# quanpn90/avsr

Measured on AMD Instinct MI355X. Metric: AV-frames/sec/GPU (fwd+bwd) on 15s clips; WER parity on LRS2 test, higher is better.
Workload: dtype bf16

## Files before the change

avsr_amd/_lib.py:

```python
import ctypes
import os

import torch

_HERE = os.path.dirname(os.path.abspath(__file__))
LIB_PATH = os.environ.get("AVSR_LIB_PATH_AB") or os.path.join(_HERE, "libavsr_hip.so")

AVSR_F32, AVSR_BF16 = 0, 1
ACT_NONE, ACT_GELU, ACT_RELU = 0, 1, 2

_c_p = ctypes.c_void_p
_i64 = ctypes.c_int64
_f = ctypes.c_float
_i = ctypes.c_int


class GemmParams(ctypes.Structure):
    _fields_ = [
        ("M", _i), ("N", _i), ("K", _i), ("batch", _i),
        ("dtype", _i), ("a_kmajor", _i), ("b_kmajor", _i), ("c_f32", _i),
        ("A", _c_p), ("lda", _i64), ("strideA", _i64),
        ("B", _c_p), ("ldb", _i64), ("strideB", _i64),
        ("C", _c_p), ("ldc", _i64), ("strideC", _i64),
        ("alpha", _f), ("beta", _f),
# ... 367 lines not shown
    global _lib
    if _lib is not None:
        return _lib
    if not os.path.exists(LIB_PATH):
        raise AvsrLibError(f"{LIB_PATH} not built: run `python -c 'import __graft_entry__ as g; g.build()'`")
    lib = ctypes.CDLL(LIB_PATH, mode=ctypes.RTLD_GLOBAL)
    for name, (argtypes, restype) in SYMBOLS.items():
        if os.environ.get("AVSR_LIB_PATH_AB") and not hasattr(lib, name):
            continue
        fn = getattr(lib, name)
        fn.argtypes = argtypes
        fn.restype = restype
    _lib = lib
    return lib


def check(rc, op):
    if rc != 0:
        raise AvsrLibError(f"{op} failed with code {rc}")


OPTIONS = {"gemm_tile": 0, "attn_sq_fwd": 1, "attn_sq_bwd": 2, "wgrad_dual": 3, "conv_192": 4, "conv_s2phase": 5,
           "conv_patch": 6, "conv_wpatch": 7, "stem_pool_2x2": 8,
           "stem_wpatch": 9, "attn_enc_fused": 10}
TILES = ["128", "256", "256x128", "128x256", "128s3", "128w8s3", "pp", "192", "192x256", "192w8s3", "64", "64s4"]
ATTN_PATHS = ["f32", "tiled", "resident", "sq", "enc"]
CONV_PATHS = ["reg", "glds", "patch", "s2", "wpatch", "stem_wpatch"]
CONV_PASSES = ["fwd", "dgrad", "wgrad"]


def set_option(name, value):
    if name == "gemm_tile" and not isinstance(value, int):
        value = 0 if value in (None, "auto") else TILES.index(value) + 1
    lib = load()
    prev = get_option(name)
    check(lib.avsr_set_option(OPTIONS[name], int(value)), f"avsr_set_option({name}, {value})")
    return prev


def get_option(name):
    return int(load().avsr_get_option(OPTIONS[name]))


_raw_stream = getattr(torch._C, "_cuda_getCurrentRawStream", None)
_get_device = getattr(torch._C, "_cuda_getDevice", None) or torch.cuda.current_device


def stream_ptr(device=None):
    if _raw_stream is not None:
        idx = _get_device() if device is None else torch.device(device).index
# ... 5 lines not shown
```

avsr_amd/csrc/conv.h:

```cpp
#pragma once
#include "gemm_core.h"
#include "gemm_glds.h"

namespace conv {
using namespace gemmcore;
using gemmg::GBK;
using gemmg::OOB;
using gemmg::bglds16;
using gemmg::make_rsrc;

struct ConvArgs {
  ConvGeom g;
  uint32_t a_bytes, b_bytes;
  const void* a; const void* b;
  int64_t a_gstride, b_gstride, c_gstride;
  int M, N, K, splits, kchunk;
  float* ws;
  Epi e;
  gemmg::BnrArgs bnr;
};

enum { K_FWD = 0, K_DGRAD = 1, K_WGRAD = 2, K_DGRAD_BNR = 3 };

struct WgradPlan { int splits, kchunk; bool slab; };
struct ConvPlan {
  int path, bm, tiles;
  int cls_bm[4], cls_tiles[4];
  uint32_t a_bytes, b_bytes;
  WgradPlan w;
  int64_t ws_floats;
};

constexpr int PATCH_ROWS = 384;
using PCfg = gemmg::GCfg<4, 1, 2, 2, 3>;
constexpr int WP_BLOCKS = 128, WP_COLS = 576, SWP_BLOCKS = 256, SWP_COLS = 392;

template <int R, int NW> struct BWgtR {
  static constexpr bool KMAJ = false;
  static constexpr int CPR = R / 8, RPP = 64 / CPR, SLOTS = GBK / RPP / NW;
  __amdgpu_buffer_rsrc_t rs; ConvGeom g;
  uint32_t vo[SLOTS];
  AVSR_DEV void init(const bf16* base, uint32_t bytes, const ConvGeom& g_, int r0, int rext, int wave, int lane) {
    rs = make_rsrc(base, bytes); g = g_;
    const int ktot = g.ktot_w;
#pragma unroll
    for (int i = 0; i < SLOTS; ++i) {
      const int pc = i * NW + wave, pk = pc * RPP + lane / CPR;
      const int r = r0 + ((lane % CPR) ^ gemmg::rswz<CPR>(pk)) * 8;
      vo[i] = r < rext ? (uint32_t)(((int64_t)pk * ktot + r) * 2) : OOB;
    }
  }
  AVSR_DEV void issue(char* img, int k0, int wave) const {
    const int ktot = g.ktot_w;
    int tap = k0 >> g.cout_shift;
    if (g.tap_step != 1) {
      const int u = (int)fdiv(tap, g.f_kw), v = tap - u * (int)g.f_kw.d;
      tap = (g.tap_kh0 + g.tap_step * u) * g.tap_kfw + g.tap_kw0 + g.tap_step * v;
    }
    const uint32_t so = (uint32_t)((((int64_t)(k0 & ((1 << g.cout_shift) - 1))) * ktot + (int64_t)tap * g.cin) * 2);
#pragma unroll
    for (int i = 0; i < SLOTS; ++i) bglds16(rs, vo[i], so, img + (i * NW + wave) * 1024);
  }
};

int igemm_f32(int kind, int bm, const ConvArgs& a, int groups, hipStream_t st);
int igemm_glds(int kind, int bm, const ConvArgs& a, int groups, hipStream_t st);
int patch_launch(int kind, const ConvArgs& a, const avsr_conv_params* p, hipStream_t st);
int wpatch_launch(const avsr_conv_params* p, hipStream_t st);
int stem_wpatch_launch(const avsr_conv_params* p, hipStream_t st);
int wgrad_reduce(float* ws, int splits, int chunks, int64_t mn, int groups, float* dw, int64_t dw_gstride, hipStream_t st);
}
```

avsr_amd/csrc/conv.hip:

```cpp
#include "conv.h"

namespace conv {
namespace {

int ilog2(int v) { int s = 0; while ((1 << s) < v) ++s; return (1 << s) == v ? s : -1; }

int make_geom(const avsr_conv_params* p, ConvGeom& g) {
  g.nimg = p->nimg; g.hin = p->hin; g.win = p->win; g.hout = p->hout; g.wout = p->wout;
  g.kh = p->kh; g.kw = p->kw; g.sh = p->sh; g.sw = p->sw; g.ph = p->ph; g.pw = p->pw;
  g.cin = p->cin; g.cout = p->cout; g.ldx = p->ldx; g.ldy = p->ldy;
  g.f_hw_out = make_fastdiv((uint32_t)(p->hout * p->wout));
  g.f_w_out = make_fastdiv((uint32_t)p->wout);
  g.f_hw_in = make_fastdiv((uint32_t)(p->hin * p->win));
  g.f_w_in = make_fastdiv((uint32_t)p->win);
  g.f_kw = make_fastdiv((uint32_t)p->kw);
  g.cin_shift = ilog2(p->cin); g.cout_shift = ilog2(p->cout);
  g.ktot_w = p->kh * p->kw * p->cin; g.tap_kfw = p->kw; g.tap_kh0 = 0; g.tap_kw0 = 0; g.tap_step = 1;
  const int ve = p->dtype == AVSR_BF16 ? 8 : 4;
  if (g.cin_shift < 0 || g.cout_shift < 0 || p->cin < ve || p->cout < ve) return AVSR_E_SHAPE;
  if (p->ldx % ve || p->ldy % ve) return AVSR_E_ALIGN;
  if (p->groups < 1 || p->ldx < (int64_t)p->groups * p->cin || p->ldy < (int64_t)p->groups * p->cout) return AVSR_E_SHAPE;
  return 0;
}

// ... 64 lines not shown
  const int64_t W = p->win, HW = (int64_t)p->hin * p->win, Wp = W + 2;
  const int64_t span = (PCfg::BM - 1) + 2 * ((PCfg::BM - 1) / W + 1) + 2 * Wp * ((PCfg::BM - 1) / HW + 1) + 2 * (Wp + 1) + 1;
  return span <= PATCH_ROWS;
}

bool wpatch_ok(const avsr_conv_params* p) {
  if (!avsr_opt(AVSR_OPT_CONV_WPATCH) || p->groups != 1 || p->splitk > 0) return false;
  if (p->kh != 3 || p->kw != 3 || p->sh != 1 || p->sw != 1 || p->ph != 1 || p->pw != 1) return false;
  if (p->cin != p->cout || p->ldx != p->cin || p->ldy != p->cout || p->hin != p->hout || p->win != p->wout) return false;
  if (p->hin != p->win) return false;
  const int64_t bytes = (int64_t)p->nimg * p->hin * p->win * p->cin * 2;
  if (bytes <= 0 || bytes >= (int64_t)OOB - (1 << 20)) return false;
  return (p->cin == 64 && p->hin == 22) || (p->cin == 128 && p->hin == 11) || (p->cin == 256 && p->hin == 6) ||
         (p->cin == 512 && p->hin == 3);
}

bool stem_wpatch_ok(const avsr_conv_params* p) {
  if (!avsr_opt(AVSR_OPT_STEM_WPATCH) || p->groups != 1 || p->splitk > 0) return false;
  if (p->cin != 8 || p->ldx != 8 || p->cout != 64 || p->ldy != 64 || p->kh != 7 || p->kw != 7) return false;
  if (p->sh != 2 || p->sw != 2 || p->ph != 3 || p->pw != 3 || p->hin != 88 || p->win != 88) return false;
  if (p->hout != 44 || p->wout != 44) return false;
  const int64_t dyb = (int64_t)p->nimg * 1936 * 128;
  return dyb > 0 && dyb < (int64_t)OOB - (1 << 20);
}

int conv_plan(const avsr_conv_params* p, int pass, ConvPlan& pl) {
  if (p->dtype != AVSR_BF16 && p->dtype != AVSR_F32) return AVSR_E_DTYPE;
  const bool bf = p->dtype == AVSR_BF16;
  pl = ConvPlan{};
  pl.path = bf ? AVSR_CONV_PATH_GLDS : AVSR_CONV_PATH_REG;
  const int64_t ktot = (int64_t)p->kh * p->kw * p->cin, ew = p->cout * ktot;
  const int64_t ex = ((int64_t)p->nimg * p->hin * p->win - 1) * p->ldx + p->cin;
  const int64_t ey = ((int64_t)p->nimg * p->hout * p->wout - 1) * p->ldy + p->cout;
  if (pass == AVSR_CONV_WGRAD) {
    set_extents(pl, bf, ey, ex);
    pl.bm = row_tile(p->cout, (int)ktot, p->groups, false);
    if (p->nimg * p->hout * p->wout == 0) return 0;
    const WgradPlan sized = wgrad_plan(p, pl.bm, bf, true);
    const int patch = !bf ? 0 : wpatch_ok(p) ? AVSR_CONV_PATH_WPATCH : stem_wpatch_ok(p) ? AVSR_CONV_PATH_STEM_WPATCH : 0;
    pl.ws_floats = patch == AVSR_CONV_PATH_WPATCH        ? (int64_t)WP_BLOCKS * 64 * WP_COLS
                   : patch == AVSR_CONV_PATH_STEM_WPATCH ? (int64_t)SWP_BLOCKS * 64 * SWP_COLS
                   : sized.slab                          ? (int64_t)p->groups * sized.splits * p->cout * ktot
                                                         : 0;
    if (p->ws && patch) pl.path = patch;
    pl.w = p->ws ? sized : wgrad_plan(p, pl.bm, bf, false);
    return 0;
  }
  const bool fwd = pass == AVSR_CONV_FWD;
  const int M = p->nimg * (fwd ? p->hout * p->wout : p->hin * p->win), N = fwd ? p->cout : p->cin;
  if (fwd) set_extents(pl, bf && (p->cin % 64) == 0, ex, ew);
  else set_extents(pl, bf && (p->cout % 64) == 0 && (p->sh == 1 || p->sh == 2) && p->sw == p->sh, ey, ew);
  if (!fwd && s2_phase(p, pl)) {
    pl.path = AVSR_CONV_PATH_S2;
    S2Class cl[4];
    s2_classes(p, cl);
    for (int q = 0; q < 4; ++q) {
      const int Mc = p->nimg * cl[q].hc * cl[q].wc;
      pl.cls_bm[q] = row_tile(Mc, N, 1, true);
      pl.cls_tiles[q] = (Mc + pl.cls_bm[q] - 1) / pl.cls_bm[q];
      pl.tiles += pl.cls_tiles[q];
    }
    return 0;
  }
  if (patch_ok(p, pl) && !(fwd && (p->bias || p->act || p->res || p->preact))) {
    pl.path = AVSR_CONV_PATH_PATCH;
    pl.bm = PCfg::BM;
  } else {
    pl.bm = row_tile(M, N, p->groups, bf);
  }
  pl.tiles = (M + pl.bm - 1) / pl.bm;
  return 0;
}

__global__ __launch_bounds__(256) void wgrad_reduce_kernel(float* ws, int splits, int chunks, int64_t mn,
                                                           float* dw, int64_t dw_gstride) {
  const int g = blockIdx.y, c = blockIdx.z;
  float* w = ws + (int64_t)g * splits * mn;
  float* d = dw + (int64_t)g * dw_gstride;
  const int nch = chunks < 0 ? -chunks : chunks;
  for (int64_t i = ((int64_t)blockIdx.x * 256 + threadIdx.x) * 4; i < mn; i += (int64_t)gridDim.x * 1024) {
    f32x4 s = {0.f, 0.f, 0.f, 0.f};
    if (chunks < 0) {
      for (int q = 0; q < nch; ++q) s += *(const f32x4*)(w + (int64_t)((int64_t)splits * q / nch) * mn + i);
    } else {
      const int s0 = (int)((int64_t)splits * c / chunks), s1 = (int)((int64_t)splits * (c + 1) / chunks);
      for (int q = s0; q < s1; ++q) s += *(const f32x4*)(w + (int64_t)q * mn + i);
      if (chunks > 1) {
        *(f32x4*)(w + (int64_t)s0 * mn + i) = s;
        continue;
// ... 1 lines not shown
    }
#pragma unroll
    for (int r = 0; r < 4; ++r) d[i + r] += s[r];
  }
}

int s2_launch(int kind, const ConvArgs& a0, const avsr_conv_params* p, const ConvPlan& pl, hipStream_t st) {
  S2Class cl[4];
  s2_classes(p, cl);
  int64_t tile_off = 0;
  for (int q = 0; q < 4; ++q) {
    const S2Class& k = cl[q];
    const int Mc = p->nimg * k.hc * k.wc;
    if (Mc == 0) continue;
    ConvArgs a = a0;
    a.g.hin = k.hc; a.g.win = k.wc; a.g.kh = k.nkh; a.g.kw = k.nkw; a.g.sh = 1; a.g.sw = 1;
    a.g.ph = k.ci; a.g.pw = k.cj;
    a.g.f_hw_in = make_fastdiv((uint32_t)(k.hc * k.wc));
    a.g.f_w_in = make_fastdiv((uint32_t)k.wc);
    a.g.f_kw = make_fastdiv((uint32_t)(k.nkw > 0 ? k.nkw : 1));
    a.g.tap_kh0 = k.kh0; a.g.tap_kw0 = k.kw0; a.g.tap_step = 2;
    a.M = Mc; a.K = k.nkh * k.nkw * p->cout; a.kchunk = a.K;
    a.e.M = Mc;
    a.e.rm_wc = k.wc; a.e.rm_hc = k.hc; a.e.rm_hin = p->hin; a.e.rm_win = p->win; a.e.rm_a = k.a; a.e.rm_b = k.b;
    if (kind >= K_DGRAD_BNR) a.bnr.ws = a0.bnr.ws + tile_off * 4 * a.N;
    tile_off += pl.cls_tiles[q];
    if (kind == K_DGRAD && a.K == 0 && a.e.beta == 1.f) continue;
    const int rc = igemm_glds(kind, pl.cls_bm[q], a, 1, st);
    if (rc) return rc;
  }
  return 0;
}

bool query_plan(const avsr_conv_params* p, int pass, ConvPlan& pl) { return p && conv_plan(p, pass, pl) == 0; }

}

int wgrad_reduce(float* ws, int splits, int chunks, int64_t mn, int groups, float* dw, int64_t dw_gstride, hipStream_t st) {
  const int xb = avsr_grid(mn / 4, 256, 1024);
  hipLaunchKernelGGL(wgrad_reduce_kernel, dim3((unsigned)xb, (unsigned)groups, (unsigned)chunks), dim3(256), 0, st, ws,
                     splits, chunks, mn, dw, dw_gstride);
  AVSR_CHECK_LAUNCH();
  if (chunks > 1) {
    hipLaunchKernelGGL(wgrad_reduce_kernel, dim3((unsigned)xb, (unsigned)groups, 1u), dim3(256), 0, st, ws, splits,
                       -chunks, mn, dw, dw_gstride);
    AVSR_CHECK_LAUNCH();
  }
  return 0;
}
}
using namespace conv;

extern "C" int avsr_conv_path(const avsr_conv_params* p, int pass) {
  if (!p || pass < AVSR_CONV_FWD || pass > AVSR_CONV_WGRAD) return AVSR_E_ARG;
  ConvGeom g;
  ConvPlan pl;
  int rc = make_geom(p, g);
  if (!rc) rc = conv_plan(p, pass, pl);
  return rc ? rc : pl.path;
}

extern "C" int avsr_conv_stat_tiles(const avsr_conv_params* p) {
  ConvPlan pl;
  return query_plan(p, AVSR_CONV_FWD, pl) ? pl.tiles : 0;
}

extern "C" int avsr_conv_bnr_tiles(const avsr_conv_params* p) {
  ConvPlan pl;
  return query_plan(p, AVSR_CONV_DGRAD, pl) ? pl.tiles : 0;
}

extern "C" int64_t avsr_conv_wgrad_ws(const avsr_conv_params* p) {
  ConvPlan pl;
  return query_plan(p, AVSR_CONV_WGRAD, pl) ? pl.ws_floats : 0;
}

extern "C" int avsr_conv_fwd(const avsr_conv_params* p, void* stream) {
  if (!p) return AVSR_E_ARG;
  ConvArgs a{};
  int rc = make_geom(p, a.g);
  if (rc) return rc;
  if (!avsr_aligned16(p->x) || !avsr_aligned16(p->w) || !avsr_aligned16(p->y)) return AVSR_E_ALIGN;
  if (p->stats && p->groups != 1) return AVSR_E_ARG;
  a.a = p->x; a.b = p->w;
  a.a_gstride = p->cin; a.b_gstride = (int64_t)p->cout * p->kh * p->kw * p->cin; a.c_gstride = p->cout;
  a.M = p->nimg * p->hout * p->wout; a.N = p->cout; a.K = p->kh * p->kw * p->cin;
  a.splits = 1; a.kchunk = a.K;
  a.e.M = a.M; a.e.N = a.N; a.e.C = p->y; a.e.ldc = p->ldy; a.e.alpha = 1.f; a.e.stats = p->stats;
  a.e.bias = p->bias; a.e.act = p->act; a.e.preact = p->preact; a.e.res = p->res; a.e.ldr = p->ldy;
  if (p->stats && (p->bias || p->act || p->res)) return AVSR_E_ARG;
  if (a.M == 0) return 0;
  ConvPlan pl;
  if ((rc = conv_plan(p, AVSR_CONV_FWD, pl))) return rc;
  a.a_bytes = pl.a_bytes; a.b_bytes = pl.b_bytes; a.e.stats_tiles = pl.tiles;
  hipStream_t st = (hipStream_t)stream;
  switch (pl.path) {
    case AVSR_CONV_PATH_REG: return igemm_f32(K_FWD, pl.bm, a, p->groups, st);
    case AVSR_CONV_PATH_PATCH: return patch_launch(K_FWD, a, p, st);
    default: return igemm_glds(K_FWD, pl.bm, a, p->groups, st);
  }
}

extern "C" int avsr_conv_bwd_data(const avsr_conv_params* p, void* stream) {
  if (!p) return AVSR_E_ARG;
  ConvArgs a{};
  int rc = make_geom(p, a.g);
  if (rc) return rc;
  if (!avsr_aligned16(p->dx) || !avsr_aligned16(p->w) || !avsr_aligned16(p->dy)) return AVSR_E_ALIGN;
  a.a = p->dy; a.b = p->w;
  a.a_gstride = p->cout; a.b_gstride = (int64_t)p->cout * p->kh * p->kw * p->cin; a.c_gstride = p->cin;
  a.M = p->nimg * p->hin * p->win; a.N = p->cin; a.K = p->kh * p->kw * p->cout;
  a.splits = 1; a.kchunk = a.K;
  a.e.M = a.M; a.e.N = a.N; a.e.C = p->dx; a.e.ldc = p->ldx; a.e.alpha = p->alpha; a.e.beta = p->beta;
  int kind = K_DGRAD;
  if (p->bnr_h) {
    if (p->dtype != AVSR_BF16 || p->groups != 1 || !p->bnr_ws || !p->bnr_scale ||
        !p->bnr_shift || !p->bnr_prelu || !p->bnr_mean || !p->bnr_invstd || (p->bnr_scale2 && !p->bnr_res) ||
        (p->bnr_scale2 && (!p->bnr_shift2 || !p->bnr_mean2 || !p->bnr_invstd2)))
      return AVSR_E_ARG;
    if (!avsr_aligned16(p->bnr_h) || (p->bnr_res && !avsr_aligned16(p->bnr_res))) return AVSR_E_ALIGN;
    a.bnr.h = (const bf16*)p->bnr_h; a.bnr.res = (const bf16*)p->bnr_res;
    a.bnr.scale = p->bnr_scale; a.bnr.shift = p->bnr_shift; a.bnr.prelu = p->bnr_prelu;
    a.bnr.mean = p->bnr_mean; a.bnr.invstd = p->bnr_invstd; a.bnr.scale2 = p->bnr_scale2;
    a.bnr.shift2 = p->bnr_shift2; a.bnr.mean2 = p->bnr_mean2; a.bnr.invstd2 = p->bnr_invstd2; a.bnr.ws = p->bnr_ws;
    kind = K_DGRAD_BNR + (p->bnr_scale2 ? 2 : p->bnr_res ? 1 : 0);
  }
  if (a.M == 0) return 0;
  ConvPlan pl;
  if ((rc = conv_plan(p, AVSR_CONV_DGRAD, pl))) return rc;
  a.a_bytes = pl.a_bytes; a.b_bytes = pl.b_bytes;
  hipStream_t st = (hipStream_t)stream;
  switch (pl.path) {
    case AVSR_CONV_PATH_REG: return igemm_f32(kind, pl.bm, a, p->groups, st);
    case AVSR_CONV_PATH_S2: return s2_launch(kind, a, p, pl, st);
    case AVSR_CONV_PATH_PATCH: return patch_launch(kind, a, p, st);
    default: return igemm_glds(kind, pl.bm, a, p->groups, st);
  }
}

extern "C" int avsr_conv_bwd_weight(const avsr_conv_params* p, void* stream) {
  if (!p) return AVSR_E_ARG;
  ConvArgs a{};
  int rc = make_geom(p, a.g);
  if (rc) return rc;
  if (!avsr_aligned16(p->x) || !avsr_aligned16(p->dy) || !p->dw) return AVSR_E_ALIGN;
  a.a = p->dy; a.b = p->x;
  const int64_t ktot = (int64_t)p->kh * p->kw * p->cin;
  a.a_gstride = p->cout; a.b_gstride = p->cin; a.c_gstride = p->cout * ktot;
  a.M = p->cout; a.N = (int)ktot; a.K = p->nimg * p->hout * p->wout;
  if (a.K == 0) return 0;
  ConvPlan pl;
  if ((rc = conv_plan(p, AVSR_CONV_WGRAD, pl))) return rc;
  hipStream_t st = (hipStream_t)stream;
  if (pl.path == AVSR_CONV_PATH_WPATCH) return wpatch_launch(p, st);
  if (pl.path == AVSR_CONV_PATH_STEM_WPATCH) return stem_wpatch_launch(p, st);
  const WgradPlan& w = pl.w;
  a.a_bytes = pl.a_bytes; a.b_bytes = pl.b_bytes;
  a.splits = w.splits; a.kchunk = w.kchunk;
// ... 15 lines not shown
```

avsr_amd/csrc/conv_igemm.hip:

```cpp
#include "conv.h"

namespace conv {
namespace {

template <typename T, typename OutT, int WM, int WN, int KIND>
__global__ __launch_bounds__(NT) void conv_kernel(ConvArgs a) {
  extern __shared__ __attribute__((aligned(16))) char smem[];
  using TL = Tile<T, WM, WN>;
  const int z = blockIdx.z, grp = z / a.splits, sp = z % a.splits;
  const int m0 = blockIdx.y * TL::BM, n0 = blockIdx.x * TL::BN;
  const T* pa = (const T*)a.a + (int64_t)grp * a.a_gstride;
  const T* pb = (const T*)a.b + (int64_t)grp * a.b_gstride;
  f32x16 acc[2][2];
  const int kbeg = sp * a.kchunk, kend = min(a.K, kbeg + a.kchunk);
  if constexpr (KIND == K_FWD) {
    LdConvK<T, TL::BM, false> la; la.p = pa; la.g = a.g; la.rext = a.M; la.K = a.K;
    LdDenseK<T, TL::BN> lb; lb.p = pb; lb.ld = a.K; lb.rext = a.N; lb.K = a.K;
    mainloop<T, WM, WN>(la, lb, m0, n0, kbeg, kend, acc, smem);
  } else if constexpr (KIND == K_DGRAD) {
    LdConvK<T, TL::BM, true> la; la.p = pa; la.g = a.g; la.rext = a.M; la.K = a.K;
    LdWgtR<T, TL::BN> lb; lb.p = pb; lb.g = a.g; lb.rext = a.N; lb.K = a.K;
    mainloop<T, WM, WN>(la, lb, m0, n0, kbeg, kend, acc, smem);
  } else {
    LdDenseR<T, TL::BM> la; la.p = pa; la.ld = a.g.ldy; la.rext = a.M; la.K = a.K;
// ... 172 lines not shown
      const uint32_t h = fdiv(rem, g.f_w_in), w = rem - h * g.f_w_in.d;
      th0[i] = h + g.ph; tw0[i] = w + g.pw;
      ro[i] = (int)(((int64_t)n * g.hout * g.wout * g.ldy + kc) * 2);
    }
  }
  AVSR_DEV void issue(char* img, int k0, int wave) const {
    const int khw = k0 >> g.cout_shift, cb = k0 & ((1 << g.cout_shift) - 1);
    const int kh = (int)fdiv(khw, g.f_kw), kw = khw - kh * (int)g.f_kw.d;
    const int ldy2 = (int)g.ldy * 2, cb2 = cb * 2;
#pragma unroll
    for (int i = 0; i < SLOTS; ++i) {
      const int th = th0[i] - kh, tw = tw0[i] - kw;
      bool ok;
      int pix;
      if (g.sh == 1) {
        ok = (unsigned)th < (unsigned)g.hout && (unsigned)tw < (unsigned)g.wout;
        pix = th * g.wout + tw;
      } else {
        ok = ((th | tw) & 1) == 0 && (unsigned)(th >> 1) < (unsigned)g.hout && (unsigned)(tw >> 1) < (unsigned)g.wout;
        pix = (th >> 1) * g.wout + (tw >> 1);
      }
      bglds16(rs, ok ? (uint32_t)(ro[i] + pix * ldy2 + cb2) : OOB, 0u, img + (i * NW + wave) * 1024);
    }
  }
};

template <int R, int NW> struct BConvR {
  static constexpr bool KMAJ = false;
  static constexpr int CPR = R / 8, RPP = 64 / CPR, SLOTS = GBK / RPP / NW;
  __amdgpu_buffer_rsrc_t rs; ConvGeom g; int kend;
  int kr[SLOTS], rk[SLOTS], rw[SLOTS], rc[SLOTS];
  AVSR_DEV void init(const bf16* base, uint32_t bytes, const ConvGeom& g_, int r0, int rext, int kend_, int wave, int lane) {
    rs = make_rsrc(base, bytes); g = g_; kend = kend_;
#pragma unroll
    for (int i = 0; i < SLOTS; ++i) {
      const int pc = i * NW + wave, pk = pc * RPP + lane / CPR;
      const int r = r0 + ((lane % CPR) ^ gemmg::rswz<CPR>(pk)) * 8;
      kr[i] = pk;
      if (r >= rext) { rk[i] = -1000000; rw[i] = 0; rc[i] = 0; continue; }
      const int c = r & ((1 << g.cin_shift) - 1), khw = r >> g.cin_shift;
      const int kh = fdiv(khw, g.f_kw);
      rk[i] = kh - g.ph; rw[i] = khw - kh * g.f_kw.d - g.pw; rc[i] = c * 2;
    }
  }
  AVSR_DEV void issue(char* img, int k0, int wave) const {
    const int ldx2 = (int)g.ldx * 2;
// ... 45 lines not shown
    gemmg::mainloop_glds<CF>(la, lb, kbeg, nk, acc, smem);
  } else if constexpr (KIND == K_DGRAD || KIND >= K_DGRAD_BNR) {
    GConvK<CF::BM, CF::NW, true> la; la.init(pa, a.g, m0, a.M, kend, wave, lane);
    GWgtR<CF::BN, CF::NW> lb; lb.init(pb, a.g, n0, a.N, kend, wave, lane);
    gemmg::mainloop_glds<CF>(la, lb, kbeg, nk, acc, smem);
  } else {
    gemmg::GDenseR<CF::BM, CF::NW> la; la.init(pa, a.g.ldy, m0, a.M, kend, wave, lane);
    GConvR<CF::BN, CF::NW> lb; lb.init(pb, a.g, n0, a.N, kend, wave, lane);
    gemmg::mainloop_glds<CF>(la, lb, kbeg, nk, acc, smem);
  }
  if constexpr (KIND >= K_DGRAD_BNR) {
    gemmg::epilogue_bnr<CF, KIND - K_DGRAD_BNR>(a.e, a.bnr, m0, n0, acc, smem);
    return;
  }
  Epi e = a.e;
  if (KIND == K_WGRAD && a.ws) e.C = a.ws + ((int64_t)grp * a.splits + sp) * a.M * a.N;
  else e.C = (OutT*)e.C + (int64_t)grp * a.c_gstride;
  if (e.res) e.res = (const bf16*)e.res + (int64_t)grp * a.c_gstride;
  if (e.preact) e.preact = (bf16*)e.preact + (int64_t)grp * a.c_gstride;
  if (e.bias) e.bias += (int64_t)grp * a.c_gstride;
  gemmg::epilogue_g<bf16, OutT, CF>(e, m0, n0, acc, smem);
}

using CCfg128 = gemmg::GCfg<2, 2, 2, 2, 2>;
using CCfg256x64 = gemmg::GCfg<4, 1, 2, 2, 2>;
using CCfg64x256 = gemmg::GCfg<1, 4, 2, 2, 2>;
using CCfg192 = gemmg::GCfg<2, 2, 3, 2, 2>;

template <typename OutT, int KIND, class CF>
int launch_glds(const ConvArgs& a, int groups, hipStream_t st) {
  const int tm = (a.M + CF::BM - 1) / CF::BM, tn = (a.N + CF::BN - 1) / CF::BN;
  if (a.e.stats && a.e.stats_tiles != tm) return AVSR_E_SHAPE;
  const long nwg = (long)tm * tn * groups * a.splits;
  if (nwg > 0x7fffffffL) return AVSR_E_SHAPE;
  hipLaunchKernelGGL((conv_glds_kernel<OutT, KIND, CF>), dim3((unsigned)nwg), dim3(CF::NTH), CF::LDS_BYTES, st, a,
                     tm, tn);
  AVSR_CHECK_LAUNCH();
  return 0;
}

template <typename OutT, int KIND>
int glds_by_tile(int bm, const ConvArgs& a, int groups, hipStream_t st) {
  if constexpr (KIND != K_WGRAD) {
    if (bm == 192) return launch_glds<OutT, KIND, CCfg192>(a, groups, st);
  }
  if (bm == 256) return launch_glds<OutT, KIND, CCfg256x64>(a, groups, st);
  if (bm == 64) return launch_glds<OutT, KIND, CCfg64x256>(a, groups, st);
  return bm == 128 ? launch_glds<OutT, KIND, CCfg128>(a, groups, st) : AVSR_E_ARG;
}

template <typename T, typename OutT, int WM, int WN, int KIND>
int launch(const ConvArgs& a, int groups, hipStream_t st) {
  using TL = Tile<T, WM, WN, KIND != K_WGRAD, KIND == K_FWD>;
  dim3 grid((a.N + TL::BN - 1) / TL::BN, (a.M + TL::BM - 1) / TL::BM, groups * a.splits);
  if (a.e.stats && a.e.stats_tiles != (int)grid.y) return AVSR_E_SHAPE;
  if (grid.y > 65535) return AVSR_E_SHAPE;
  hipLaunchKernelGGL((conv_kernel<T, OutT, WM, WN, KIND>), grid, dim3(NT), TL::LDS_BYTES, st, a);
  AVSR_CHECK_LAUNCH();
  return 0;
}

template <int KIND>
int f32_by_tile(int bm, const ConvArgs& a, int groups, hipStream_t st) {
  if (bm == 256) return launch<float, float, 4, 1, KIND>(a, groups, st);
  if (bm == 64) return launch<float, float, 1, 4, KIND>(a, groups, st);
  return bm == 128 ? launch<float, float, 2, 2, KIND>(a, groups, st) : AVSR_E_ARG;
}

}

int igemm_f32(int kind, int bm, const ConvArgs& a, int groups, hipStream_t st) {
  if (kind == K_FWD) return f32_by_tile<K_FWD>(bm, a, groups, st);
  if (kind == K_DGRAD) return f32_by_tile<K_DGRAD>(bm, a, groups, st);
  return kind == K_WGRAD ? f32_by_tile<K_WGRAD>(bm, a, groups, st) : AVSR_E_ARG;
}

int igemm_glds(int kind, int bm, const ConvArgs& a, int groups, hipStream_t st) {
  switch (kind) {
    case K_FWD: return glds_by_tile<bf16, K_FWD>(bm, a, groups, st);
    case K_DGRAD: return glds_by_tile<bf16, K_DGRAD>(bm, a, groups, st);
    case K_WGRAD: return glds_by_tile<float, K_WGRAD>(bm, a, groups, st);
    case K_DGRAD_BNR: return glds_by_tile<bf16, K_DGRAD_BNR>(bm, a, groups, st);
    case K_DGRAD_BNR + 1: return glds_by_tile<bf16, K_DGRAD_BNR + 1>(bm, a, groups, st);
    case K_DGRAD_BNR + 2: return glds_by_tile<bf16, K_DGRAD_BNR + 2>(bm, a, groups, st);
    default: return AVSR_E_ARG;
  }
}
}
```

avsr_amd/csrc/gemm_core.h:

```cpp
#pragma once
#include "common.h"

namespace gemmcore {

constexpr int BKE = 32, NT = 256;

template <typename T> struct V { static constexpr int VE = 16 / (int)sizeof(T); static constexpr int ROW = BKE + VE; };

AVSR_DEV void zero(v16& v) { v.w[0] = v.w[1] = v.w[2] = v.w[3] = 0u; }

struct ConvGeom {
  int nimg, hin, win, hout, wout;
  int kh, kw, sh, sw, ph, pw;
  int cin, cout;
  int64_t ldx, ldy;
  FastDiv f_hw_out, f_w_out;
  FastDiv f_hw_in, f_w_in;
  FastDiv f_kw;
  int cin_shift, cout_shift;
  int ktot_w, tap_kfw, tap_kh0, tap_kw0, tap_step;
};

template <typename T, int R> struct LdDenseK {
  static constexpr bool KMAJ = true;
// ... 234 lines not shown
          }
        }
    }
    if (more) {
      lstore<T, TL::BM, LA::KMAJ>(lA + (cur ^ 1) * TL::SA, ra, tid);
      lstore<T, TL::BN, LB::KMAJ>(lB + (cur ^ 1) * TL::SB, rb, tid);
    }
    __syncthreads();
  }
}

struct Epi {
  int M, N;
  void* C; int64_t ldc;
  float alpha, beta;
  const float* bias;
  int act, bwd, atomic;
  void* preact;
  const void* res; int64_t ldr;
  const void* gate;
  float drop_p; uint64_t seed; uint64_t drop_base;
  float* stats;
  int stats_tiles;
  int rm_wc, rm_hc, rm_hin, rm_win, rm_a, rm_b;
  float* colsum;
};

AVSR_DEV int epi_row(const Epi& e, int r) {
  if (e.rm_wc == 0) return r;
  const int q = r / e.rm_wc, j = r - q * e.rm_wc;
  const int n = q / e.rm_hc, i = q - n * e.rm_hc;
  return (n * e.rm_hin + 2 * i + e.rm_a) * e.rm_win + 2 * j + e.rm_b;
}

AVSR_DEV int acc_row(int wm, int i, int r, int lane) { return wm * 64 + i * 32 + (r & 3) + 8 * (r >> 2) + 4 * (lane >> 5); }
AVSR_DEV int acc_col(int wn, int j, int lane) { return wn * 64 + j * 32 + (lane & 31); }

template <typename T, typename OutT, int NE>
AVSR_DEV void epi_elems(const Epi& e, int row, int col, const float* v_in) {
  OutT* C = (OutT*)e.C;
  const T* R = (const T*)e.res;
  T* P = (T*)e.preact;
  const T* G = (const T*)e.gate;
  const int64_t off = (int64_t)row * e.ldc + col;
  if (e.atomic) {
#pragma unroll
    for (int q = 0; q < NE; ++q)
      if (col + q < e.N) atomicAdd((float*)C + off + q, e.alpha * v_in[q]);
    return;
  }
#pragma unroll
  for (int q = 0; q < NE; ++q) {
    if (col + q >= e.N) break;
    float v = e.alpha * v_in[q];
    const uint64_t didx = e.drop_base + (uint64_t)row * (uint64_t)e.N + col + q;
// ... 240 lines not shown
```

avsr_amd/csrc/version.hip:

```cpp
#include <atomic>

#include "common.h"

extern "C" const char* avsr_version(void) { return "avsr_hip 0.2.0 gfx950"; }

#ifndef AVSR_AB_ATTN_ENC_FUSED
#define AVSR_AB_ATTN_ENC_FUSED 1
#endif

namespace {
std::atomic<int64_t> g_opt[AVSR_OPT_COUNT] = {{0}, {1}, {0}, {1}, {1}, {1}, {1}, {1}, {1}, {1}, {AVSR_AB_ATTN_ENC_FUSED}};

bool opt_valid(int option, int64_t v) {
  switch (option) {
    case AVSR_OPT_GEMM_TILE: return v >= 0 && v <= AVSR_TILE_COUNT;
    case AVSR_OPT_ATTN_SQ_BWD: return v == 0;
    case AVSR_OPT_ATTN_SQ_FWD:
    case AVSR_OPT_WGRAD_DUAL:
    case AVSR_OPT_CONV_192:
    case AVSR_OPT_CONV_S2PHASE:
    case AVSR_OPT_CONV_PATCH:
    case AVSR_OPT_CONV_WPATCH:
    case AVSR_OPT_STEM_POOL_2X2:
    case AVSR_OPT_STEM_WPATCH:
    case AVSR_OPT_ATTN_ENC_FUSED: return v == 0 || v == 1;
    default: return false;
  }
}
}

int64_t avsr_opt(int option) { return g_opt[option].load(std::memory_order_relaxed); }

extern "C" int avsr_set_option(int option, int64_t value) {
  if (!opt_valid(option, value)) return AVSR_E_ARG;
  g_opt[option].store(value, std::memory_order_relaxed);
  return 0;
}

extern "C" int64_t avsr_get_option(int option) {
  if (option < 0 || option >= AVSR_OPT_COUNT) return -1;
  return avsr_opt(option);
}
```

avsr_amd/ops.py:

```python
import ctypes
import os

import torch

from . import _lib as L

_DT = {torch.float32: L.AVSR_F32, torch.bfloat16: L.AVSR_BF16}

PROBE = {}

SLAB_PAD = 1088


def slab_ws(batch, splitk, M, N):
    return batch * splitk * (M * N + SLAB_PAD)


def dtype_code(t):
    try:
        return _DT[t.dtype]
    except KeyError:
        raise L.AvsrLibError(f"unsupported dtype {t.dtype}")


# ... 210 lines not shown
        p = L.ConvParams()
        p.dtype = dtype
        p.nimg, p.hin, p.win, p.cin = self.nimg, self.hin, self.win, self.cin
        p.hout, p.wout, p.cout = self.hout, self.wout, self.cout
        p.kh, p.kw, p.sh, p.sw, p.ph, p.pw = self.kh, self.kw, self.sh, self.sw, self.ph, self.pw
        p.groups, p.ldx, p.ldy = self.groups, self.ldx, self.ldy
        p.alpha, p.beta = 1.0, 0.0
        return p

    @property
    def out_pixels(self):
        return self.nimg * self.hout * self.wout

    @property
    def in_pixels(self):
        return self.nimg * self.hin * self.win


def conv_stat_tiles(g, dtype):
    p = g.params(dtype)
    return L.load().avsr_conv_stat_tiles(ctypes.byref(p))


def conv_path(g, dtype, pass_, *, bias=False, act=L.ACT_NONE, preact=False, res=False, ws=False, splitk=0):
    p = g.params(_DT.get(dtype, dtype))
    p.act, p.splitk = act, splitk
    for name, on in (("bias", bias), ("preact", preact), ("res", res), ("ws", ws)):
        setattr(p, name, 16 if on else None)
    rc = L.load().avsr_conv_path(ctypes.byref(p), L.CONV_PASSES.index(pass_))
    if not 0 <= rc < len(L.CONV_PATHS):
        L.check(rc, "avsr_conv_path")
    return L.CONV_PATHS[rc]


def conv_fwd(g, x, w, y, stats=None, bias=None, act=L.ACT_NONE, preact=None, res=None):
    p = g.params(dtype_code(x))
    assert x.dtype == w.dtype == y.dtype and x.is_cuda
    if stats is not None:
        tiles = L.load().avsr_conv_stat_tiles(ctypes.byref(p))
        if stats.dtype != torch.float32 or stats.numel() < g.groups * g.cout * tiles * 3 or not stats.is_contiguous():
            raise ValueError(f"conv_fwd stats: need fp32 [{g.cout}, {tiles}, 3], got {tuple(stats.shape)}")
    p.x, p.w, p.y = x.data_ptr(), w.data_ptr(), y.data_ptr()
    p.stats = None if stats is None else stats.data_ptr()
    p.bias = None if bias is None else bias.data_ptr()
    p.act = act
    p.preact = None if preact is None else preact.data_ptr()
    p.res = None if res is None else res.data_ptr()
    p._keep = [t for t in (x, w, y, stats, bias, preact, res) if t is not None]
    L.check(L.load().avsr_conv_fwd(ctypes.byref(p), L.stream_ptr()), "avsr_conv_fwd")
    return y
# ... 703 lines not shown
```

include/avsr_hip.h:

```cpp
#ifndef AVSR_HIP_H
#define AVSR_HIP_H

#include <stdint.h>

#ifdef __cplusplus
extern "C" {
#endif

enum { AVSR_F32 = 0, AVSR_BF16 = 1 };
enum { AVSR_ACT_NONE = 0, AVSR_ACT_GELU = 1, AVSR_ACT_RELU = 2 };
enum { AVSR_E_SHAPE = 1001, AVSR_E_ALIGN = 1002, AVSR_E_DTYPE = 1003, AVSR_E_ARG = 1004 };

const char* avsr_version(void);

enum {
  AVSR_OPT_GEMM_TILE = 0,
  AVSR_OPT_ATTN_SQ_FWD = 1,
  AVSR_OPT_ATTN_SQ_BWD = 2,
  AVSR_OPT_WGRAD_DUAL = 3,
  AVSR_OPT_CONV_192 = 4,
  AVSR_OPT_CONV_S2PHASE = 5,
  AVSR_OPT_CONV_PATCH = 6,
  AVSR_OPT_CONV_WPATCH = 7,
  AVSR_OPT_STEM_POOL_2X2 = 8,
  AVSR_OPT_STEM_WPATCH = 9,
  AVSR_OPT_ATTN_ENC_FUSED = 10,
  AVSR_OPT_COUNT = 11
};
enum {
  AVSR_TILE_128 = 0, AVSR_TILE_256 = 1, AVSR_TILE_256x128 = 2, AVSR_TILE_128x256 = 3, AVSR_TILE_128s3 = 4,
  AVSR_TILE_128w8s3 = 5, AVSR_TILE_PP = 6, AVSR_TILE_192 = 7, AVSR_TILE_192x256 = 8, AVSR_TILE_192w8s3 = 9,
  AVSR_TILE_64 = 10, AVSR_TILE_64s4 = 11, AVSR_TILE_COUNT = 12
};
int avsr_set_option(int option, int64_t value);
int64_t avsr_get_option(int option);

typedef struct {
  int M, N, K, batch;
  int dtype;
  int a_kmajor, b_kmajor;
  int c_f32;
  const void* A; int64_t lda, strideA;
  const void* B; int64_t ldb, strideB;
  void* C;       int64_t ldc, strideC;
  float alpha, beta;
  const float* bias;
  int act;
  int epi_bwd;
  void* preact;
  const void* res;  int64_t ldr, strideR;
// ... 37 lines not shown
  const void* x; const void* w; void* y;
  void* dx; const void* dy; float* dw;
  float* stats;
  float alpha, beta;
  int splitk;
  const float* bias; int act; void* preact; const void* res;
  float* ws;
  const void* bnr_h; const void* bnr_res;
  const float* bnr_scale; const float* bnr_shift; const float* bnr_prelu;
  const float* bnr_mean; const float* bnr_invstd;
  const float* bnr_scale2; const float* bnr_shift2; const float* bnr_mean2; const float* bnr_invstd2;
  float* bnr_ws;
} avsr_conv_params;

int avsr_conv_fwd(const avsr_conv_params* p, void* stream);
int avsr_conv_bwd_data(const avsr_conv_params* p, void* stream);
int avsr_conv_bwd_weight(const avsr_conv_params* p, void* stream);
int avsr_conv_stat_tiles(const avsr_conv_params* p);
int avsr_conv_bnr_tiles(const avsr_conv_params* p);
int64_t avsr_conv_wgrad_ws(const avsr_conv_params* p);
enum { AVSR_CONV_FWD = 0, AVSR_CONV_DGRAD = 1, AVSR_CONV_WGRAD = 2 };
enum {
  AVSR_CONV_PATH_REG = 0, AVSR_CONV_PATH_GLDS = 1, AVSR_CONV_PATH_PATCH = 2, AVSR_CONV_PATH_S2 = 3,
  AVSR_CONV_PATH_WPATCH = 4, AVSR_CONV_PATH_STEM_WPATCH = 5
};
int avsr_conv_path(const avsr_conv_params* p, int pass);

typedef struct {
  int dtype, rows, N;
  float eps;
  const void* x; int64_t ldx;
  void* y; int64_t ldy;
  const float* gamma; const float* beta;
  float* mean; float* rstd;
  const void* dy; int64_t lddy;
  void* dx; int64_t lddx;
  const void* dres; int64_t lddres;
  float* dgamma; float* dbeta;
  float* ws;
  void* g; int64_t ldg; float drop_p; uint64_t seed; float* db;
} avsr_layernorm_params;
#define AVSR_LN_BLOCKS 256
#define AVSR_LN_WS(N) (AVSR_LN_BLOCKS * 2 * (N))
#define AVSR_LN_WS3(N) (AVSR_LN_BLOCKS * 3 * (N))
int avsr_layernorm_fwd(const avsr_layernorm_params* p, void* stream);
int avsr_layernorm_bwd(const avsr_layernorm_params* p, void* stream);

// ... 406 lines not shown
```

Baseline: 146,700.

## Add edge-class conv path that skips zero-padding taps for small 3x3 convs

Adds a new conv path for 3x3 stride-1 pad-1 convolutions on small spatial maps. Output pixels are split into up to nine classes (interior, edges, corners), and each class is run as an implicit GEMM over only the kernel taps that land inside the image, so no MACs are spent on zero padding. The path is taken only when the estimated saved work is large enough and the batch is big, and it is on by default. It adds a multi-class launch, a generalized epilogue row map using fastdiv, and a small change to the tap remap in the weight loader. The risk is less efficient tiles for the small edge classes, plus per-block class lookup overhead.

After: 147,900, median of 6. No clear change (+0.8%).

```diff
diff --git a/avsr_amd/_lib.py b/avsr_amd/_lib.py
--- a/avsr_amd/_lib.py
+++ b/avsr_amd/_lib.py
@@ -413,10 +413,10 @@
 
 OPTIONS = {"gemm_tile": 0, "attn_sq_fwd": 1, "attn_sq_bwd": 2, "wgrad_dual": 3, "conv_192": 4, "conv_s2phase": 5,
            "conv_patch": 6, "conv_wpatch": 7, "stem_pool_2x2": 8,
-           "stem_wpatch": 9, "attn_enc_fused": 10}
+           "stem_wpatch": 9, "attn_enc_fused": 10, "conv_edge": 11}
 TILES = ["128", "256", "256x128", "128x256", "128s3", "128w8s3", "pp", "192", "192x256", "192w8s3", "64", "64s4"]
 ATTN_PATHS = ["f32", "tiled", "resident", "sq", "enc"]
-CONV_PATHS = ["reg", "glds", "patch", "s2", "wpatch", "stem_wpatch"]
+CONV_PATHS = ["reg", "glds", "patch", "s2", "wpatch", "stem_wpatch", "edge"]
 CONV_PASSES = ["fwd", "dgrad", "wgrad"]
 
 
diff --git a/avsr_amd/csrc/conv.h b/avsr_amd/csrc/conv.h
--- a/avsr_amd/csrc/conv.h
+++ b/avsr_amd/csrc/conv.h
@@ -23,9 +23,17 @@
 enum { K_FWD = 0, K_DGRAD = 1, K_WGRAD = 2, K_DGRAD_BNR = 3 };
 
 struct WgradPlan { int splits, kchunk; bool slab; };
+struct EdgeClass {
+  int rows, K, blk0, pt0;
+  uint32_t m_hw, m_w;
+  uint16_t hc, wc, h0, w0;
+  uint8_t s_hw, s_w, kh0, kw0, nkh, nkw;
+};
+struct EdgeTab { int ncls, blocks; EdgeClass c[9]; };
 struct ConvPlan {
   int path, bm, tiles;
   int cls_bm[4], cls_tiles[4];
+  EdgeTab edge;
   uint32_t a_bytes, b_bytes;
   WgradPlan w;
   int64_t ws_floats;
@@ -53,7 +61,7 @@
   AVSR_DEV void issue(char* img, int k0, int wave) const {
     const int ktot = g.ktot_w;
     int tap = k0 >> g.cout_shift;
-    if (g.tap_step != 1) {
+    if (g.tap_step != 1 || g.tap_kh0 != 0 || g.tap_kw0 != 0 || g.tap_kfw != (int)g.f_kw.d) {
       const int u = (int)fdiv(tap, g.f_kw), v = tap - u * (int)g.f_kw.d;
       tap = (g.tap_kh0 + g.tap_step * u) * g.tap_kfw + g.tap_kw0 + g.tap_step * v;
     }
@@ -65,6 +73,7 @@
 
 int igemm_f32(int kind, int bm, const ConvArgs& a, int groups, hipStream_t st);
 int igemm_glds(int kind, int bm, const ConvArgs& a, int groups, hipStream_t st);
+int edge_launch(int kind, int bm, const ConvArgs& a, const EdgeTab& t, hipStream_t st);
 int patch_launch(int kind, const ConvArgs& a, const avsr_conv_params* p, hipStream_t st);
 int wpatch_launch(const avsr_conv_params* p, hipStream_t st);
 int stem_wpatch_launch(const avsr_conv_params* p, hipStream_t st);
diff --git a/avsr_amd/csrc/conv.hip b/avsr_amd/csrc/conv.hip
--- a/avsr_amd/csrc/conv.hip
+++ b/avsr_amd/csrc/conv.hip
@@ -110,6 +110,48 @@
   if (p->hout != 44 || p->wout != 44) return false;
   const int64_t dyb = (int64_t)p->nimg * 1936 * 128;
   return dyb > 0 && dyb < (int64_t)OOB - (1 << 20);
+}
+
+bool edge_ok(const avsr_conv_params* p, const ConvPlan& pl, bool fwd) {
+  if (!avsr_opt(AVSR_OPT_CONV_EDGE) || !pl.a_bytes || p->groups != 1) return false;
+  if (p->kh != 3 || p->kw != 3 || p->sh != 1 || p->sw != 1 || p->ph != 1 || p->pw != 1) return false;
+  if (p->hin != p->hout || p->win != p->wout || p->hin < 2 || p->win < 2 || p->hin > 32767 || p->win > 32767) return false;
+  if (fwd && (p->stats || p->bias || p->act || p->res || p->preact)) return false;
+  const int64_t H = p->hin, W = p->win;
+  if (5 * (3 * H - 2) * (3 * W - 2) > 36 * H * W) return false;
+  return p->nimg >= 192;
+}
+
+void edge_plan(const avsr_conv_params* p, bool fwd, ConvPlan& pl) {
+  const int H = p->hin, W = p->win, N = fwd ? p->cout : p->cin, kc = fwd ? p->cin : p->cout;
+  auto seg = [&](int L, int q, int (&o)[4]) {
+    o[0] = q == 0 ? 0 : q == 1 ? 1 : L - 1;
+    o[1] = q == 1 ? L - 2 : 1;
+    o[3] = q == 1 ? 3 : 2;
+    o[2] = q == 1 ? 0 : ((q == 0) == fwd ? 1 : 0);
+  };
+  EdgeTab& t = pl.edge;
+  t.ncls = 0;
+  for (int nt = 9; nt >= 4; --nt)
+    for (int q = 0; q < 9; ++q) {
+      int r[4], c[4];
+      seg(H, q / 3, r); seg(W, q % 3, c);
+      if (r[3] * c[3] != nt || r[1] <= 0 || c[1] <= 0) continue;
+      EdgeClass& k = t.c[t.ncls++];
+      k.h0 = (uint16_t)r[0]; k.hc = (uint16_t)r[1]; k.kh0 = (uint8_t)r[2]; k.nkh = (uint8_t)r[3];
+      k.w0 = (uint16_t)c[0]; k.wc = (uint16_t)c[1]; k.kw0 = (uint8_t)c[2]; k.nkw = (uint8_t)c[3];
+      k.rows = p->nimg * r[1] * c[1]; k.K = nt * kc;
+      const FastDiv fhw = make_fastdiv((uint32_t)(r[1] * c[1])), fw = make_fastdiv((uint32_t)c[1]);
+      k.m_hw = fhw.m; k.s_hw = (uint8_t)fhw.s; k.m_w = fw.m; k.s_w = (uint8_t)fw.s;
+    }
+  pl.bm = row_tile(p->nimg * H * W, N, 1, true);
+  const int bn = pl.bm == 256 ? 64 : pl.bm == 64 ? 256 : 128, tn = (N + bn - 1) / bn;
+  t.blocks = 0; pl.tiles = 0;
+  for (int i = 0; i < t.ncls; ++i) {
+    const int tm = (t.c[i].rows + pl.bm - 1) / pl.bm;
+    t.c[i].blk0 = t.blocks; t.c[i].pt0 = pl.tiles;
+    t.blocks += tm * tn; pl.tiles += tm;
+  }
 }
 
 int conv_plan(const avsr_conv_params* p, int pass, ConvPlan& pl) {
@@ -153,6 +195,10 @@
   if (patch_ok(p, pl) && !(fwd && (p->bias || p->act || p->res || p->preact))) {
     pl.path = AVSR_CONV_PATH_PATCH;
     pl.bm = PCfg::BM;
+  } else if (edge_ok(p, pl, fwd)) {
+    pl.path = AVSR_CONV_PATH_EDGE;
+    edge_plan(p, fwd, pl);
+    return 0;
   } else {
     pl.bm = row_tile(M, N, p->groups, bf);
   }
@@ -200,7 +246,8 @@
     a.g.tap_kh0 = k.kh0; a.g.tap_kw0 = k.kw0; a.g.tap_step = 2;
     a.M = Mc; a.K = k.nkh * k.nkw * p->cout; a.kchunk = a.K;
     a.e.M = Mc;
-    a.e.rm_wc = k.wc; a.e.rm_hc = k.hc; a.e.rm_hin = p->hin; a.e.rm_win = p->win; a.e.rm_a = k.a; a.e.rm_b = k.b;
+    a.e.rm_wc = k.wc; a.e.rm_fhw = a.g.f_hw_in; a.e.rm_fw = a.g.f_w_in; a.e.rm_hin = p->hin; a.e.rm_win = p->win;
+    a.e.rm_a = k.a; a.e.rm_b = k.b; a.e.rm_step = 2;
     if (kind >= K_DGRAD_BNR) a.bnr.ws = a0.bnr.ws + tile_off * 4 * a.N;
     tile_off += pl.cls_tiles[q];
     if (kind == K_DGRAD && a.K == 0 && a.e.beta == 1.f) continue;
@@ -239,8 +286,11 @@
 }
 
 extern "C" int avsr_conv_stat_tiles(const avsr_conv_params* p) {
-  ConvPlan pl;
-  return query_plan(p, AVSR_CONV_FWD, pl) ? pl.tiles : 0;
+  if (!p) return 0;
+  avsr_conv_params q = *p;
+  if (!q.stats) q.stats = reinterpret_cast<float*>(16);
+  ConvPlan pl;
+  return query_plan(&q, AVSR_CONV_FWD, pl) ? pl.tiles : 0;
 }
 
 extern "C" int avsr_conv_bnr_tiles(const avsr_conv_params* p) {
@@ -275,6 +325,7 @@
   switch (pl.path) {
     case AVSR_CONV_PATH_REG: return igemm_f32(K_FWD, pl.bm, a, p->groups, st);
     case AVSR_CONV_PATH_PATCH: return patch_launch(K_FWD, a, p, st);
+    case AVSR_CONV_PATH_EDGE: return edge_launch(K_FWD, pl.bm, a, pl.edge, st);
     default: return igemm_glds(K_FWD, pl.bm, a, p->groups, st);
   }
 }
@@ -312,6 +363,7 @@
     case AVSR_CONV_PATH_REG: return igemm_f32(kind, pl.bm, a, p->groups, st);
     case AVSR_CONV_PATH_S2: return s2_launch(kind, a, p, pl, st);
     case AVSR_CONV_PATH_PATCH: return patch_launch(kind, a, p, st);
+    case AVSR_CONV_PATH_EDGE: return edge_launch(kind, pl.bm, a, pl.edge, st);
     default: return igemm_glds(kind, pl.bm, a, p->groups, st);
   }
 }
diff --git a/avsr_amd/csrc/conv_igemm.hip b/avsr_amd/csrc/conv_igemm.hip
--- a/avsr_amd/csrc/conv_igemm.hip
+++ b/avsr_amd/csrc/conv_igemm.hip
@@ -218,6 +218,29 @@
       }
       bglds16(rs, ok ? (uint32_t)(ro[i] + pix * ldy2 + cb2) : OOB, 0u, img + (i * NW + wave) * 1024);
     }
+  }
+};
+
+template <int R, int NW> struct BWgtK {
+  static constexpr bool KMAJ = true;
+  static constexpr int SLOTS = R / 8 / NW;
+  __amdgpu_buffer_rsrc_t rs; ConvGeom g;
+  uint32_t vo[SLOTS];
+  AVSR_DEV void init(const bf16* base, uint32_t bytes, const ConvGeom& g_, int r0, int rext, int wave, int lane) {
+    rs = make_rsrc(base, bytes); g = g_;
+#pragma unroll
+    for (int i = 0; i < SLOTS; ++i) {
+      const int pc = i * NW + wave, pr = pc * 8 + (lane >> 3);
+      const int c = (lane & 7) ^ ((pr >> 1) & 7);
+      vo[i] = r0 + pr < rext ? (uint32_t)(((int64_t)(r0 + pr) * g.ktot_w + c * 8) * 2) : OOB;
+    }
+  }
+  AVSR_DEV void issue(char* img, int k0, int wave) const {
+    const int t = k0 >> g.cin_shift, u = (int)fdiv(t, g.f_kw), v = t - u * (int)g.f_kw.d;
+    const int tap = (g.tap_kh0 + g.tap_step * u) * g.tap_kfw + g.tap_kw0 + g.tap_step * v;
+    const uint32_t so = (uint32_t)((tap * g.cin + (k0 & ((1 << g.cin_shift) - 1))) * 2);
+#pragma unroll
+    for (int i = 0; i < SLOTS; ++i) bglds16(rs, vo[i], so, img + (i * NW + wave) * 1024);
   }
 };
 
@@ -309,6 +332,47 @@
   gemmg::epilogue_g<bf16, OutT, CF>(e, m0, n0, acc, smem);
 }
 
+template <int KIND, class CF>
+__global__ __launch_bounds__(CF::NTH, CF::MINB) void conv_edge_kernel(ConvArgs a, EdgeTab t, int tiles_n) {
+  extern __shared__ __attribute__((aligned(16))) char smem[];
+  const int bid = blockIdx.x;
+  int ci = 0;
+  for (int i = 1; i < t.ncls; ++i) ci = bid >= t.c[i].blk0 ? i : ci;
+  const EdgeClass& k = t.c[ci];
+  const int tiles_m = (k.rows + CF::BM - 1) / CF::BM;
+  int tm, tn, z;
+  gemmg::tile_of(gemmg::xcd_remap(bid - k.blk0, tiles_m * tiles_n), tiles_m, tiles_n, tm, tn, z);
+  const int m0 = tm * CF::BM, n0 = tn * CF::BN, nk = k.K / GBK;
+  const int lane = threadIdx.x & 63, wave = __builtin_amdgcn_readfirstlane(threadIdx.x >> 6);
+  ConvGeom g = a.g;
+  const FastDiv fhw = {(uint32_t)k.hc * k.wc, k.m_hw, k.s_hw}, fw = {k.wc, k.m_w, k.s_w};
+  g.f_kw = FastDiv{k.nkw, k.nkw == 3 ? 0x55555556u : 1u, k.nkw - 1u};
+  g.tap_kh0 = k.kh0; g.tap_kw0 = k.kw0;
+  f32x4 acc[CF::TM][CF::TN];
+  if constexpr (KIND == K_FWD) {
+    g.f_hw_out = fhw; g.f_w_out = fw; g.ph = 1 - k.h0 - k.kh0; g.pw = 1 - k.w0 - k.kw0;
+    BConvK<CF::BM, CF::NW> la; la.init((const bf16*)a.a, a.a_bytes, g, m0, k.rows, wave, lane);
+    BWgtK<CF::BN, CF::NW> lb; lb.init((const bf16*)a.b, a.b_bytes, g, n0, a.N, wave, lane);
+    gemmg::mainloop_glds<CF>(la, lb, 0, nk, acc, smem);
+  } else {
+    g.f_hw_in = fhw; g.f_w_in = fw; g.ph = 1 + k.h0 - k.kh0; g.pw = 1 + k.w0 - k.kw0;
+    BConvKT<CF::BM, CF::NW> la; la.init((const bf16*)a.a, a.a_bytes, g, m0, k.rows, wave, lane);
+    BWgtR<CF::BN, CF::NW> lb; lb.init((const bf16*)a.b, a.b_bytes, g, n0, a.N, wave, lane);
+    gemmg::mainloop_glds<CF>(la, lb, 0, nk, acc, smem);
+  }
+  Epi e = a.e;
+  e.M = k.rows;
+  e.rm_wc = k.wc; e.rm_fhw = fhw; e.rm_fw = fw; e.rm_hin = g.hin; e.rm_win = g.win;
+  e.rm_a = k.h0; e.rm_b = k.w0; e.rm_step = 1;
+  if constexpr (KIND >= K_DGRAD_BNR) {
+    gemmg::BnrArgs b = a.bnr;
+    b.ws += (int64_t)k.pt0 * 4 * a.N;
+    gemmg::epilogue_bnr<CF, KIND - K_DGRAD_BNR>(e, b, m0, n0, acc, smem);
+  } else {
+    gemmg::epilogue_g<bf16, bf16, CF>(e, m0, n0, acc, smem);
+  }
+}
+
 using CCfg128 = gemmg::GCfg<2, 2, 2, 2, 2>;
 using CCfg256x64 = gemmg::GCfg<4, 1, 2, 2, 2>;
 using CCfg64x256 = gemmg::GCfg<1, 4, 2, 2, 2>;
@@ -336,6 +400,25 @@
   return bm == 128 ? launch_glds<OutT, KIND, CCfg128>(a, groups, st) : AVSR_E_ARG;
 }
 
+template <int KIND, class CF>
+int launch_edge(const ConvArgs& a, const EdgeTab& t, hipStream_t st) {
+  const int tn = (a.N + CF::BN - 1) / CF::BN;
+  int tiles = 0;
+  for (int i = 0; i < t.ncls; ++i) tiles += (t.c[i].rows + CF::BM - 1) / CF::BM;
+  if (t.ncls < 1 || t.ncls > 9 || !a.a_bytes || !a.b_bytes || t.blocks != tiles * tn) return AVSR_E_ARG;
+  if (a.e.stats) return AVSR_E_ARG;
+  hipLaunchKernelGGL((conv_edge_kernel<KIND, CF>), dim3((unsigned)t.blocks), dim3(CF::NTH), CF::LDS_BYTES, st, a, t, tn);
+  AVSR_CHECK_LAUNCH();
+  return 0;
+}
+
+template <int KIND>
+int edge_by_tile(int bm, const ConvArgs& a, const EdgeTab& t, hipStream_t st) {
+  if (bm == 192) return launch_edge<KIND, CCfg192>(a, t, st);
+  if (bm == 256) return launch_edge<KIND, CCfg256x64>(a, t, st);
+  return bm == 128 ? launch_edge<KIND, CCfg128>(a, t, st) : AVSR_E_ARG;
+}
+
 template <typename T, typename OutT, int WM, int WN, int KIND>
 int launch(const ConvArgs& a, int groups, hipStream_t st) {
   using TL = Tile<T, WM, WN, KIND != K_WGRAD, KIND == K_FWD>;
@@ -373,4 +456,15 @@
     default: return AVSR_E_ARG;
   }
 }
-}
+
+int edge_launch(int kind, int bm, const ConvArgs& a, const EdgeTab& t, hipStream_t st) {
+  switch (kind) {
+    case K_FWD: return edge_by_tile<K_FWD>(bm, a, t, st);
+    case K_DGRAD: return edge_by_tile<K_DGRAD>(bm, a, t, st);
+    case K_DGRAD_BNR: return edge_by_tile<K_DGRAD_BNR>(bm, a, t, st);
+    case K_DGRAD_BNR + 1: return edge_by_tile<K_DGRAD_BNR + 1>(bm, a, t, st);
+    case K_DGRAD_BNR + 2: return edge_by_tile<K_DGRAD_BNR + 2>(bm, a, t, st);
+    default: return AVSR_E_ARG;
+  }
+}
+}
diff --git a/avsr_amd/csrc/gemm_core.h b/avsr_amd/csrc/gemm_core.h
--- a/avsr_amd/csrc/gemm_core.h
+++ b/avsr_amd/csrc/gemm_core.h
@@ -280,15 +280,16 @@
   float drop_p; uint64_t seed; uint64_t drop_base;
   float* stats;
   int stats_tiles;
-  int rm_wc, rm_hc, rm_hin, rm_win, rm_a, rm_b;
+  int rm_wc, rm_hin, rm_win, rm_a, rm_b, rm_step;
+  FastDiv rm_fhw, rm_fw;
   float* colsum;
 };
 
 AVSR_DEV int epi_row(const Epi& e, int r) {
   if (e.rm_wc == 0) return r;
-  const int q = r / e.rm_wc, j = r - q * e.rm_wc;
-  const int n = q / e.rm_hc, i = q - n * e.rm_hc;
-  return (n * e.rm_hin + 2 * i + e.rm_a) * e.rm_win + 2 * j + e.rm_b;
+  const int n = (int)fdiv(r, e.rm_fhw), rem = r - n * (int)e.rm_fhw.d;
+  const int i = (int)fdiv(rem, e.rm_fw), j = rem - i * e.rm_wc;
+  return (n * e.rm_hin + e.rm_step * i + e.rm_a) * e.rm_win + e.rm_step * j + e.rm_b;
 }
 
 AVSR_DEV int acc_row(int wm, int i, int r, int lane) { return wm * 64 + i * 32 + (r & 3) + 8 * (r >> 2) + 4 * (lane >> 5); }
diff --git a/avsr_amd/csrc/version.hip b/avsr_amd/csrc/version.hip
--- a/avsr_amd/csrc/version.hip
+++ b/avsr_amd/csrc/version.hip
@@ -9,7 +9,7 @@
 #endif
 
 namespace {
-std::atomic<int64_t> g_opt[AVSR_OPT_COUNT] = {{0}, {1}, {0}, {1}, {1}, {1}, {1}, {1}, {1}, {1}, {AVSR_AB_ATTN_ENC_FUSED}};
+std::atomic<int64_t> g_opt[AVSR_OPT_COUNT] = {{0}, {1}, {0}, {1}, {1}, {1}, {1}, {1}, {1}, {1}, {AVSR_AB_ATTN_ENC_FUSED}, {1}};
 
 bool opt_valid(int option, int64_t v) {
   switch (option) {
@@ -23,7 +23,8 @@
     case AVSR_OPT_CONV_WPATCH:
     case AVSR_OPT_STEM_POOL_2X2:
     case AVSR_OPT_STEM_WPATCH:
-    case AVSR_OPT_ATTN_ENC_FUSED: return v == 0 || v == 1;
+    case AVSR_OPT_ATTN_ENC_FUSED:
+    case AVSR_OPT_CONV_EDGE: return v == 0 || v == 1;
     default: return false;
   }
 }
diff --git a/avsr_amd/ops.py b/avsr_amd/ops.py
--- a/avsr_amd/ops.py
+++ b/avsr_amd/ops.py
@@ -256,10 +256,11 @@
     return L.load().avsr_conv_stat_tiles(ctypes.byref(p))
 
 
-def conv_path(g, dtype, pass_, *, bias=False, act=L.ACT_NONE, preact=False, res=False, ws=False, splitk=0):
+def conv_path(g, dtype, pass_, *, bias=False, act=L.ACT_NONE, preact=False, res=False, ws=False, splitk=0,
+              stats=False):
     p = g.params(_DT.get(dtype, dtype))
     p.act, p.splitk = act, splitk
-    for name, on in (("bias", bias), ("preact", preact), ("res", res), ("ws", ws)):
+    for name, on in (("bias", bias), ("preact", preact), ("res", res), ("ws", ws), ("stats", stats)):
         setattr(p, name, 16 if on else None)
     rc = L.load().avsr_conv_path(ctypes.byref(p), L.CONV_PASSES.index(pass_))
     if not 0 <= rc < len(L.CONV_PATHS):
diff --git a/include/avsr_hip.h b/include/avsr_hip.h
--- a/include/avsr_hip.h
+++ b/include/avsr_hip.h
@@ -25,7 +25,8 @@
   AVSR_OPT_STEM_POOL_2X2 = 8,
   AVSR_OPT_STEM_WPATCH = 9,
   AVSR_OPT_ATTN_ENC_FUSED = 10,
-  AVSR_OPT_COUNT = 11
+  AVSR_OPT_CONV_EDGE = 11,
+  AVSR_OPT_COUNT = 12
 };
 enum {
   AVSR_TILE_128 = 0, AVSR_TILE_256 = 1, AVSR_TILE_256x128 = 2, AVSR_TILE_128x256 = 3, AVSR_TILE_128s3 = 4,
@@ -109,7 +110,7 @@
 enum { AVSR_CONV_FWD = 0, AVSR_CONV_DGRAD = 1, AVSR_CONV_WGRAD = 2 };
 enum {
   AVSR_CONV_PATH_REG = 0, AVSR_CONV_PATH_GLDS = 1, AVSR_CONV_PATH_PATCH = 2, AVSR_CONV_PATH_S2 = 3,
-  AVSR_CONV_PATH_WPATCH = 4, AVSR_CONV_PATH_STEM_WPATCH = 5
+  AVSR_CONV_PATH_WPATCH = 4, AVSR_CONV_PATH_STEM_WPATCH = 5, AVSR_CONV_PATH_EDGE = 6
 };
 int avsr_conv_path(const avsr_conv_params* p, int pass);
 
```
